# matchylabs/matchy

Hardware: AMD Instinct MI355X
Metric: log GB/s scanned (matchy match hot path, 100K IoCs) (higher is better)
Workload: dtype u8

## Files before the change

### matchy_amd/csrc/engine.cpp

```cpp
#include "engine.h"
#include "batch_reader.h"
#include "distinct.h"
#include "tally.h"
#include "unicode_lower.h"

#include <dlfcn.h>

#include <algorithm>
#include <chrono>
#include <cstdio>
#include <cstdlib>
#include <cstring>
#include <stdexcept>
#include <unordered_set>

#include "hashes.h"

namespace mxy {

void check_launch(const char* kernel) {
    const hipError_t e = hipGetLastError();
    if (e != hipSuccess) throw HipError{std::string("launch of ") + kernel + ": " + hipGetErrorString(e)};
}

// ... 191 lines not shown
                    launch_ip_leaf(ip_nodes.p, img.node_count, ip_l24.p, ctr.p + 1, (uint32_t)n_leaf, leaf_node.p, ip_leaf.p, nullptr);
                    MXY_HIP(hipDeviceSynchronize());
                    view.ip_leaf = ip_leaf.p;
                    bytes_uploaded += n_leaf * 256 * sizeof(uint2);
                }
                view.ip_l24 = ip_l24.p;
                bytes_uploaded += ((size_t)1 << 24) * sizeof(uint2);
                MXY_HIP(hipMemcpy(bm.data(), ip_bm24.p, bm.size() * 4, hipMemcpyDeviceToHost));
                have24 = true;
            } catch (const HipError&) {
                (void)hipGetLastError();
                ip_l24.free(); ip_leaf.free(); ip_bm24.free();
                view.ip_l24 = nullptr; view.ip_leaf = nullptr;
                std::fill(bm.begin(), bm.end(), 0u);
            }
        }
        if (!have24) {
            if (img.node_count > 0) {
                auto set_range = [&](uint32_t first, uint32_t count) {
                    for (uint32_t v = first; v < first + count;) {
                        if ((v & 31) == 0 && v + 32 <= first + count) { bm[v >> 5] = 0xFFFFFFFFu; v += 32; }
                        else { bm[v >> 5] |= 1u << (v & 31); ++v; }
                    }
                };
                struct Frame { uint32_t node, prefix, depth; };
                std::vector<Frame> st;
                st.push_back({v4_start, 0u, 0u});
                while (!st.empty()) {
                    const Frame f = st.back();
                    st.pop_back();
                    const uint2 nd = nodes[f.node];
                    for (uint32_t bit = 0; bit < 2; ++bit) {
                        const uint32_t rec = bit ? nd.y : nd.x;
                        const uint32_t depth = f.depth + 1;
                        const uint32_t prefix = f.prefix | (bit << (24 - depth));
                        if (rec == img.node_count) continue;
                        if (rec < img.node_count) {
                            if (depth == 24) set_range(prefix, 1);
                            else st.push_back({rec, prefix, depth});
                        } else if (rec - img.node_count >= 16) {
                            set_range(prefix, 1u << (24 - depth));
                        }
                    }
                }
            }
            ip_bm24.upload(bm);
        }
        view.ip_bm24 = ip_bm24.p;
        {
            uint64_t set = 0;
            for (uint32_t wv : bm) set += (uint64_t)__builtin_popcount(wv);
            view.ip_bm24_permille = (uint32_t)(set * 1000 / ((uint64_t)bm.size() * 32));
            view.ip_bm24_any = set ? 1u : 0u;
        }
        bytes_uploaded += bm.size() * 4;
    }
    if (img.has_literal) {
        std::vector<LitSlot> slots;
        uint32_t mask;
        img.build_lit_table(slots, mask);
        lit_slots.upload(slots);
        const uint8_t* pool = img.bytes.data() + img.lh_off + img.lh_strings_offset;
        std::vector<uint8_t> pv(pool, pool + img.lh_strings_size);
        lit_pool.upload(pv);
        {
            size_t bits = (size_t)1 << 22;
            size_t live = 0;
            for (const LitSlot& sl : slots) live += sl.str_off != 0xFFFFFFFFu;
            while (bits < live * 64 && bits < ((size_t)1 << 31)) bits <<= 1;
            std::vector<uint32_t> bm(bits / 32, 0u);
            const uint32_t bmask = (uint32_t)(bits - 1);
            for (const LitSlot& sl : slots) {
                if (sl.str_off == 0xFFFFFFFFu || (size_t)sl.str_off + 2 > pv.size()) continue;
                const size_t kl = (size_t)pv[sl.str_off] | ((size_t)pv[sl.str_off + 1] << 8);
                if ((size_t)sl.str_off + 2 + kl > pv.size()) continue;
                uint64_t lane[4] = {0, 0, 0, 0};
                memcpy(lane, pv.data() + sl.str_off + 2, std::min<size_t>(kl, 32));
                const uint32_t b = name_hash31(lane[0], lane[1], lane[2], lane[3], (uint32_t)kl) & bmask;
                bm[b >> 5] |= 1u << (b & 31);
            }
            lit_bm.upload(bm);
            view.lit_bm = lit_bm.p; view.lit_bm_mask = bmask;
            bytes_uploaded += bm.size() * 4;
        }
        uint32_t max_len = 0;
        for (const LitSlot& sl : slots)
            if (sl.str_off != 0xFFFFFFFFu && (size_t)sl.str_off + 2 <= pv.size()) max_len = std::max<uint32_t>(max_len, (uint32_t)pv[sl.str_off] | ((uint32_t)pv[sl.str_off + 1] << 8));
        view.lit_max_len = max_len;
        view.lit_slots = lit_slots.p; view.lit_mask = mask; view.has_literal = 1;
        view.lit_pool = lit_pool.p; view.lit_pool_size = img.lh_strings_size;
        bytes_uploaded += slots.size() * sizeof(LitSlot) + pv.size();
    }
    if (img.has_glob) {
        const uint8_t* pgp = img.bytes.data() + img.pg_off;
        std::vector<uint8_t> pv(pgp, pgp + img.pg_len);
        pv.resize((pv.size() + 3) & ~(size_t)3, 0);
        pg.upload(pv);
        std::vector<uint32_t> off, ids;
        img.build_lit2pat(off, ids);
        if (ids.empty()) ids.push_back(0);
        lit2pat_off.upload(off);
        lit2pat.upload(ids);
        auto r32 = [&](size_t o) { uint32_t v; memcpy(&v, pgp + o, 4); return v; };
        view.pg = pg.p; view.pg_len = (uint32_t)img.pg_len; view.has_glob = 1;
        view.ac_start = r32(20); view.ac_size = r32(24);
        view.patterns_off = r32(36); view.pattern_count = r32(32);
        uint32_t unaligned = r32(40) + r32(44);
        view.wild_off = unaligned + (8 - unaligned % 8) % 8;
        view.wild_count = r32(60);
        view.glob_seg_off = r32(104);
        view.glob_max_segs = 1;
        for (uint32_t pid = 0; pid < view.pattern_count; ++pid) view.glob_max_segs = std::max<uint32_t>(view.glob_max_segs, r32((size_t)view.glob_seg_off + (size_t)pid * 8 + 4) & 0xFFFFu);
        view.lit2pat_off = lit2pat_off.p; view.lit2pat = lit2pat.p; view.n_ac_lits = (uint32_t)off.size() - 1;
        {
            std::vector<uint32_t> nx, noff;
            std::vector<uint8_t> cls;
            uint32_t k = 0;
            size_t limit = (size_t)8 << 30;
            if (const char* env = getenv("MATCHY_AMD_DFA_MAX_MB")) limit = (size_t)atoll(env) << 20;
            bool alnum_literal = true;
            view.ac_alnum = 1;
            if (img.build_ac_dfa(nx, cls, k, noff, limit, &alnum_literal)) {
                view.ac_alnum = alnum_literal ? 1u : 0u;
                if (img.match_mode == 1) for (int c = 'A'; c <= 'Z'; ++c) cls[c] = cls[c + 32];
                dfa.upload(nx); dfa_node.upload(noff); dfa_cls.upload(cls);
                view.dfa = dfa.p; view.dfa_node = dfa_node.p; view.dfa_cls = dfa_cls.p; view.dfa_k = k;
                view.dfa_states = (uint32_t)noff.size();
                bytes_uploaded += nx.size() * 4 + noff.size() * 4 + 256;
            }
        }
        bytes_uploaded += pv.size() + (off.size() + ids.size()) * 4;
        if (view.dfa && view.wild_count == 0 && view.pattern_count && !getenv("MATCHY_AMD_NO_SUFFIX_FILTER")) {
            const bool ci_db = img.match_mode == 1;
            bool ok = true;
            int first = -1;
            uint32_t dots = 0;
            std::vector<std::pair<uint32_t, uint32_t>> lits;
            for (uint32_t pid = 0; pid < view.pattern_count && ok; ++pid) {
                const size_t io = (size_t)view.glob_seg_off + (size_t)pid * 8;
                const uint32_t firsth = r32(io), count = r32(io + 4) & 0xFFFFu;
                if (count != 2 || (size_t)firsth + 24 > img.pg_len) { ok = false; break; }
                const uint8_t* h0 = pgp + firsth;
                const uint8_t* h1 = pgp + firsth + 12;
                uint32_t dlen, doff;
                memcpy(&dlen, h1 + 4, 4); memcpy(&doff, h1 + 8, 4);
                if (h0[0] != 1 || h1[0] != 0 || (size_t)doff + dlen > img.pg_len) { ok = false; break; }
                if (dlen < 3) continue;
                const uint8_t* l = pgp + doff;
                const int fb = ci_db ? (int)ascii_lower1(l[0]) : (int)l[0];
                if (first < 0) first = fb;
                if (fb != first) { ok = false; break; }
                uint32_t d = 0;
                for (uint32_t k = 0; k < dlen; ++k) d += (ci_db ? ascii_lower1(l[k]) : l[k]) == (uint32_t)first;
                if (d > 32) { ok = false; break; }
                dots |= 1u << (d - 1);
                if (dlen <= 31) lits.push_back({doff, dlen});
            }
            if (ok && first >= 0 && __builtin_popcount(dots) <= 4) {
                size_t bits = (size_t)1 << 16;
                while (bits < lits.size() * 64 && bits < ((size_t)1 << 31)) bits <<= 1;
                std::vector<uint32_t> bm(bits / 32, 0u);
                const uint32_t bmask = (uint32_t)(bits - 1);
                for (auto& ol : lits) {
                    uint64_t lane[4] = {0, 0, 0, 0};
                    memcpy(lane, pgp + ol.first, ol.second);
                    if (ci_db) for (uint64_t& w : lane) w = ascii_lower8(w);
// ... 1053 lines not shown
```

### matchy_amd/csrc/engine.h

```cpp
#pragma once
#include <hip/hip_runtime.h>

#include <memory>
#include <mutex>
#include <string>
#include <vector>

#include "db_image.h"
#include "hip_owners.h"
#include "inflate.h"
#include "line_index.h"
#include "result_layout.h"
#include "scan_types.h"
#include "segments.h"

namespace mxy {

int anchor_blocks_per_cu();
int validate_blocks_per_cu(bool ac);
void launch_anchor(const TokParams& p, const DevDb& db, int grid, hipStream_t stream);
void launch_validate_dom(const TokParams& p, const DevDb& db, int grid, hipStream_t stream);
void launch_validate_misc(const TokParams& p, const DevDb& db, int grid, hipStream_t stream);
void launch_rare(const TokParams& p, const DevDb& db, int grid, hipStream_t stream);
void launch_lookup(const LookupParams& p, const DevDb& db, int grid, hipStream_t stream);
void launch_lookup_early_glob(const LookupParams& p, const DevDb& db, int grid, hipStream_t stream);
void launch_lookup_ip(const LookupParams& p, const DevDb& db, int grid, bool dense, hipStream_t stream);
void launch_lookup_spill(const LookupParams& p, const DevDb& db, hipStream_t stream);
uint32_t spill_threads();
void launch_ip_l24(const uint2* nodes, uint32_t node_count, uint32_t v4_start, uint2* l24, uint32_t* bm24, uint32_t* n_undecided, hipStream_t s);
void launch_ip_leaf(const uint2* nodes, uint32_t node_count, uint2* l24, uint32_t* next, uint32_t n_leaf, uint32_t* leaf_node, uint2* leaf, hipStream_t s);

class DistinctSet;
class HitTally;
struct TallyEntry;

struct PslHost {
    std::vector<std::string> suffixes;
    std::vector<PslSlot> slots;
    std::vector<uint8_t> pool;
    std::vector<uint32_t> bloom;
    std::vector<uint2> tld_tab;
    uint32_t mask = 0, max_tld_len = 0, max_suffix_len = 0;
    uint32_t tld_first[8] = {0};
    static const PslHost& get();
};

struct DeviceDb {
    int device = 0;
    DevDb view{};
    DevBuf<uint2> ip_nodes, ip_l1, ip_l24, ip_leaf;
    DevBuf<uint32_t> ip_bm24, lit_bm, sfx_bm;
    DevBuf<uint2> tld_tab;
    DevBuf<uint32_t> dfa, dfa_node;
    DevBuf<uint8_t> dfa_cls;
    DevBuf<LitSlot> lit_slots;
    DevBuf<uint8_t> lit_pool, pg, psl_pool;
    DevBuf<uint32_t> lit2pat_off, lit2pat, bloom;
    DevBuf<uint32_t> lit_offsets, glob_offsets;
    DevBuf<PslSlot> psl_slots;
    DevBuf<uint32_t> lc_map;
    DevBuf<uint2> lc_ign, lc_cased;
    uint32_t n_lit_offsets = 0, n_glob_offsets = 0;
    size_t bytes_uploaded = 0;
    void upload(const DbImage& img, int dev);
};

struct ScanTiming { float anchor_ms = 0, validate_ms = 0, rare_ms = 0, lookup_ms = 0, total_ms = 0; int slices = 1; };

enum HitMode { HITS_NONE = 0, HITS_FINAL = 1, HITS_RAW = 2 };

struct ScanOutput {
    std::vector<Candidate> cands;
    std::vector<Hit> hits;
    std::vector<uint32_t> ids;
    const FinalHit* fin = nullptr;
    const uint32_t* fin_ids = nullptr;
    const long long* fin_offs = nullptr;
    size_t n_fin = 0, n_fin_ids = 0;
    const uint2* c4 = nullptr;
    size_t n_c4 = 0;
    uint64_t lines = 0;
    uint32_t n_cand = 0, n_hits = 0;
    uint64_t by_type[IT_COUNT] = {0};
    bool has_lines = false;
    const LineRec* fin_lines = nullptr;
    const LineRec* c4_lines = nullptr;
    uint64_t lines_with_matches = 0;
    bool has_segments = false;
    const SegmentRec* segments = nullptr;
    size_t n_segments = 0;
    const uint32_t* seg_of_fin = nullptr;
    const uint32_t* seg_of_c4 = nullptr;
    std::vector<SegmentRec> seg_own;
    std::vector<uint32_t> seg_of_own;
};

namespace pins {
bool acquire(uintptr_t a, uintptr_t b);
void release(uintptr_t a, uintptr_t b);
int add_caller(const void* ptr, size_t bytes);
void remove_caller(const void* ptr);
}

template <class Hit, class Off, class OffOut>
void append_shifted(const Hit* hits, size_t n_hits, const uint32_t* ids, const Off* offs, size_t n_ids, uint32_t base,
                    std::vector<Hit>& all_hits, std::vector<uint32_t>& all_ids, std::vector<OffOut>& all_offs) {
    const uint32_t id_shift = (uint32_t)all_ids.size();
    for (size_t i = 0; i < n_hits; ++i) {
        Hit h = hits[i];
        h.start += base;
        if (h.kind == 3) h.value += id_shift;
        all_hits.push_back(h);
    }
    all_ids.insert(all_ids.end(), ids, ids + n_ids);
    all_offs.insert(all_offs.end(), offs, offs + n_ids);
}

struct ScanRequest {
    const uint8_t* ptr = nullptr;
    uint32_t len = 0;
    bool lookup = false;
    bool host_mirror = false;
    bool fork = false;
    int slices = 0;
    bool compact = false;
    bool lines = false;
};

template <class Line>
void append_shifted_lines(const Line* lines, size_t n, uint32_t base, uint32_t line_base, std::vector<Line>& all) {
    for (size_t i = 0; i < n; ++i) {
        Line l = lines[i];
        l.line += line_base; l.line_start += base; l.line_end += base;
        all.push_back(l);
// ... 155 lines not shown
```

### matchy_amd/csrc/hashes.h

```cpp
#pragma once
#include <cstddef>
#include <cstdint>

#if defined(__HIPCC__)
#include <hip/hip_runtime.h>
#define MXY_HD __host__ __device__ inline __attribute__((always_inline))
#else
#define MXY_HD inline
#endif

namespace mxy {

MXY_HD uint64_t rotl64(uint64_t x, int r) { return (x << r) | (x >> (64 - r)); }

template <class Fetch>
MXY_HD uint64_t xxh64_fetch(Fetch f, size_t len, uint64_t seed) {
    const uint64_t P1 = 11400714785074694791ULL, P2 = 14029467366897019727ULL, P3 = 1609587929392839161ULL,
                   P4 = 9650029242287828579ULL, P5 = 2870177450012600261ULL;
    auto rd64 = [&](size_t o) {
        uint64_t v = 0;
        for (int k = 7; k >= 0; --k) v = (v << 8) | (uint64_t)f(o + k);
        return v;
    };
    auto rd32 = [&](size_t o) {
// ... 50 lines not shown
            q += 32;
        } while (q <= limit);
        h = rotl64(v1, 1) + rotl64(v2, 7) + rotl64(v3, 12) + rotl64(v4, 18);
        h = merge(h, v1); h = merge(h, v2); h = merge(h, v3); h = merge(h, v4);
    } else {
        h = seed + P5;
    }
    h += (uint64_t)len;
    if (len >= 8) {
        const uint64_t last = rd64(len - 8);
        if (len < 32) {
            const uint64_t w0 = rd64(0), w1 = rd64(len >= 16 ? 8 : len - 8), w2 = rd64(len >= 24 ? 16 : len - 8);
            h ^= round(0, w0); h = rotl64(h, 27) * P1 + P4;
            if (len >= 16) { h ^= round(0, w1); h = rotl64(h, 27) * P1 + P4; }
            if (len >= 24) { h ^= round(0, w2); h = rotl64(h, 27) * P1 + P4; }
            q = len & ~(size_t)7;
        } else {
            while (q + 8 <= len) { h ^= round(0, rd64(q)); h = rotl64(h, 27) * P1 + P4; q += 8; }
        }
        size_t r = len - q;
        uint64_t tail = r ? last >> (8 * (8 - r)) : 0;
        if (r >= 4) { h ^= (tail & 0xFFFFFFFFull) * P1; h = rotl64(h, 23) * P2 + P3; tail >>= 32; r -= 4; }
        for (; r; --r) { h ^= (tail & 0xFF) * P5; h = rotl64(h, 11) * P1; tail >>= 8; }
    } else {
        if (q + 4 <= len) { h ^= rd32(q) * P1; h = rotl64(h, 23) * P2 + P3; q += 4; }
        while (q < len) { h ^= (uint64_t)(FOLD ? ascii_lower1(p[q]) : (uint32_t)p[q]) * P5; h = rotl64(h, 11) * P1; ++q; }
    }
    h ^= h >> 33; h *= P2; h ^= h >> 29; h *= P3; h ^= h >> 32;
    return h;
}

struct Xxh64Stream {
    static constexpr uint64_t P1 = 11400714785074694791ULL, P2 = 14029467366897019727ULL, P3 = 1609587929392839161ULL,
                              P4 = 9650029242287828579ULL, P5 = 2870177450012600261ULL;
    uint64_t v1, v2, v3, v4, lane[4] = {0, 0, 0, 0}, cur = 0, total = 0;
    uint32_t nlane = 0, ncur = 0;
    MXY_HD explicit Xxh64Stream(uint64_t seed) : v1(seed + P1 + P2), v2(seed + P2), v3(seed), v4(seed - P1) {}
    static MXY_HD uint64_t round(uint64_t acc, uint64_t in) { acc += in * P2; acc = rotl64(acc, 31); return acc * P1; }
    static MXY_HD uint64_t merge(uint64_t acc, uint64_t val) { val = round(0, val); acc ^= val; return acc * P1 + P4; }
    MXY_HD void push(uint32_t byte) {
        cur |= (uint64_t)(byte & 0xFF) << (8 * ncur);
        ++total;
        if (++ncur == 8) {
            lane[nlane] = cur; cur = 0; ncur = 0;
            if (++nlane == 4) {
                v1 = round(v1, lane[0]); v2 = round(v2, lane[1]); v3 = round(v3, lane[2]); v4 = round(v4, lane[3]);
                nlane = 0;
            }
        }
    }
    MXY_HD uint64_t finish(uint64_t seed) const {
        uint64_t h;
        if (total >= 32) {
            h = rotl64(v1, 1) + rotl64(v2, 7) + rotl64(v3, 12) + rotl64(v4, 18);
            h = merge(h, v1); h = merge(h, v2); h = merge(h, v3); h = merge(h, v4);
        } else {
            h = seed + P5;
        }
        h += total;
        for (uint32_t k = 0; k < nlane; ++k) { h ^= round(0, lane[k]); h = rotl64(h, 27) * P1 + P4; }
        uint64_t rest = cur;
        uint32_t n = ncur;
        if (n >= 4) { h ^= (rest & 0xFFFFFFFFull) * P1; h = rotl64(h, 23) * P2 + P3; rest >>= 32; n -= 4; }
        for (; n; --n) { h ^= (rest & 0xFF) * P5; h = rotl64(h, 11) * P1; rest >>= 8; }
        h ^= h >> 33; h *= P2; h ^= h >> 29; h *= P3; h ^= h >> 32;
        return h;
    }
};

MXY_HD uint32_t name_hash31(uint64_t l0, uint64_t l1, uint64_t l2, uint64_t l3, uint32_t n) {
    const uint64_t lane[4] = {l0, l1, l2, l3};
    uint32_t h = n * 0x9E3779B1u + 0x7F4A7C15u;
    for (int k = 0; k < 4; ++k) {
        const int rem = (int)n - 8 * k;
        const uint64_t m = rem >= 8 ? ~0ull : rem <= 0 ? 0ull : ((1ull << (8 * rem)) - 1ull);
        const uint64_t v = lane[k] & m;
        h = (h ^ (uint32_t)v) * 0x85EBCA6Bu; h ^= h >> 15;
        h = (h ^ (uint32_t)(v >> 32)) * 0xC2B2AE35u; h ^= h >> 13;
    }
    h *= 0x27D4EB2Fu; h ^= h >> 16;
    return h;
}

MXY_HD uint64_t fx_u32(uint32_t v) { return rotl64((uint64_t)v * 0xf1357aea2e62a9c5ULL, 26); }

constexpr uint32_t TLD_TAB_BITS = 11;
MXY_HD uint32_t tld_tab_slot(uint32_t lo, uint32_t hi24) { return ((lo ^ (hi24 * 0x9E3779B1u)) * 0x85EBCA6Bu) >> (32 - TLD_TAB_BITS); }

MXY_HD uint32_t tld_hash8(uint32_t lo, uint32_t hi) {
    uint32_t h = (lo * 0x9E3779B1u) ^ (hi * 0x85EBCA6Bu);
    h ^= h >> 16; h *= 0x7FEB352Du; h ^= h >> 15;
    return h;
}

MXY_HD uint64_t psl_hash_init() { return 0xcbf29ce484222325ULL; }
MXY_HD uint64_t psl_hash_step(uint64_t h, uint8_t b) { return (h ^ b) * 0x100000001b3ULL; }
MXY_HD uint64_t psl_hash_finish(uint64_t h) { h ^= h >> 29; h *= 0xbf58476d1ce4e5b9ULL; h ^= h >> 32; return h; }

}
```

### matchy_amd/csrc/scan_types.h

```cpp
#pragma once
#include <hip/hip_runtime.h>

#include <cstdint>

namespace mxy {

enum ItemType : uint8_t {
    IT_DOMAIN = 0, IT_EMAIL = 1, IT_IPV4 = 2, IT_IPV6 = 3, IT_MD5 = 4, IT_SHA1 = 5, IT_SHA256 = 6,
    IT_SHA384 = 7, IT_SHA512 = 8, IT_BITCOIN = 9, IT_ETHEREUM = 10, IT_MONERO = 11, IT_COUNT = 12
};
enum ExtractFlags : uint32_t {
    EX_DOMAINS = 1, EX_EMAILS = 2, EX_IPV4 = 4, EX_IPV6 = 8, EX_HASHES = 16, EX_BITCOIN = 32, EX_ETHEREUM = 64,
    EX_MONERO = 128, EX_ALL = 255
};

struct Candidate {
    uint32_t start;
    uint32_t len_type;
    uint32_t v4;
    uint32_t pad;
};
constexpr uint32_t CAND_NO_GLOB = 1, CAND_GLOB = 2;

enum RareKind : uint32_t { RARE_V6 = 0, RARE_AT = 1, RARE_TOK = 2, HEAVY_B58 = 3, HEAVY_BECH32 = 4, HEAVY_ETH = 5, HEAVY_XMR = 6, RARE_DOM = 7 };
struct RareAnchor {
    uint32_t pos;
    uint32_t len_kind;
};

struct Hit {
    uint32_t cand;
    uint32_t a;
    uint32_t ids_off;
    uint16_t n_globs;
    uint8_t kind;
    uint8_t prefix_len;
    uint32_t start;
    uint32_t len_type;
};

struct LitSlot { uint64_t hash; uint32_t str_off; uint32_t pattern_id; };
struct PslSlot { uint64_t hash; uint32_t off; uint32_t len; };

struct DevDb {
    const uint2* ip_nodes;
    uint32_t ip_bm24_permille;
    uint32_t ip_bm24_any;
    const uint32_t* ip_bm24;
    const uint2* ip_l1;
    const uint2* ip_l24;
    const uint2* ip_leaf;
    uint32_t node_count;
    uint32_t ip_version;
    uint32_t v4_start_node;
    uint32_t has_ip;
    const LitSlot* lit_slots;
    uint32_t lit_mask;
    uint32_t has_literal;
    const uint32_t* lit_bm;
    uint32_t lit_bm_mask;
    const uint8_t* lit_pool;
    uint32_t lit_pool_size;
    uint32_t lit_max_len;
    const uint8_t* pg;
    uint32_t pg_len;
    uint32_t has_glob;
    uint32_t ac_start, ac_size;
    uint32_t patterns_off, pattern_count;
    uint32_t wild_off, wild_count;
    uint32_t glob_seg_off;
    uint32_t glob_max_segs;
    const uint32_t* dfa;
    const uint8_t* dfa_cls;
    const uint32_t* dfa_node;
    uint32_t dfa_k;
    uint32_t dfa_states;
    const uint32_t* sfx_bm;
    uint32_t sfx_mask;
    uint32_t sfx_first;
    uint32_t sfx_dots;
    const uint32_t* lit2pat_off;
    const uint32_t* lit2pat;
    uint32_t n_ac_lits;
    uint32_t ac_alnum;
    const PslSlot* psl_slots;
    uint32_t psl_mask;
    const uint8_t* psl_pool;
    const uint32_t* tld_bloom;
    uint32_t max_tld_len;
    uint32_t max_suffix_len;
    const uint2* tld_tab;
    uint32_t tld_first[8];
    uint32_t ci;
    const uint32_t* lc_map;
    uint32_t lc_n;
    const uint2* lc_ign;
    uint32_t lc_n_ign;
    const uint2* lc_cased;
    uint32_t lc_n_cased;
};

constexpr uint32_t DFA_LDS_ENTRIES = 8192;
constexpr uint32_t DFA_LDS_ENTRIES_GLOB = 2048;
constexpr uint32_t DFA_LDS_ENTRIES_VAL = 2048;
constexpr uint32_t TLD_BLOOM_BITS = 32768;
constexpr uint32_t TLD_BLOOM_WORDS = TLD_BLOOM_BITS / 32;

struct ScanCounters {
    alignas(128) unsigned long long lines;
    uint32_t cand_true;
    uint32_t hits_true;
    uint32_t error;
    uint32_t reserved0;
    alignas(128) uint32_t n_cand;
    alignas(128) uint32_t n_cand_a;
    alignas(128) uint32_t n_cand_m;
    uint32_t n_cand_d;
    uint32_t n_cand_r;
    alignas(128) uint32_t n_dom;
    alignas(128) uint32_t n_rare;
    alignas(128) uint32_t n_rare_dom;
    alignas(128) uint32_t n_tok;
    alignas(128) uint32_t n_heavy;
    alignas(128) uint32_t n_hits;
    uint32_t n_ids;
    alignas(128) uint32_t n_final;
    uint32_t n_final_ids;
    uint32_t n_c4;
    alignas(128) uint32_t chains_done;
    uint32_t arrive_wgs[3];
    alignas(128) uint32_t n_glob_work;
    uint32_t n_glob_work_d;
    uint32_t n_spill;
};

struct FinalHit {
    uint32_t start;
    uint32_t len_type;
    uint32_t value;
    uint8_t kind, prefix_len;
    uint16_t n_ids;
};

// ... 119 lines not shown
```

### matchy_amd/csrc/validate_kernels.hip

```cpp
#include <hip/hip_runtime.h>

#include <cstdlib>

#include "hashes.h"
#include "scan_types.h"

#include "device_shared.h"
#include "domain_planes.h"

namespace mxy {


struct BackReader {
    const uint8_t* p;
    uint32_t pos;
    uint32_t cb;
    uint32_t k;
    uint64_t cur, nxt;
    __device__ __forceinline__ static uint64_t load8(const uint8_t* a) { uint64_t v; __builtin_memcpy(&v, a, 8); return v; }
    __device__ __forceinline__ void init(const uint8_t* base, uint32_t q) {
        p = base; pos = q; cb = 0; k = 0; cur = 0; nxt = 0;
        if (q >= 16) { cb = q - 8; k = 8; cur = load8(p + cb); nxt = load8(p + cb - 8); }
    }
    __device__ __forceinline__ uint32_t next() {
// ... 662 lines not shown
    for (int i = 0; i < NL; ++i) {
#pragma unroll
        for (int bb = 0; bb < 4; ++bb) {
            const uint32_t j = 4 * i + bb;
            if (j < nbytes) dec[zeros + nbytes - 1 - j] = (uint8_t)(L[i] >> (8 * bb));
        }
    }
    return zeros + nbytes;
}
__device__ bool val_btc_base58(const uint8_t* s, uint32_t n, uint8_t* dec) {
    const uint32_t dl = d_base58_decode<12>(s, n, dec);
    if (dl < 5) return false;
    Sha256 h1, h2;
    h1.hash(dec, dl - 4);
    uint32_t w[16];
#pragma unroll
    for (int i = 0; i < 8; ++i) w[i] = h1.h[i];
    w[8] = 0x80000000u;
#pragma unroll
    for (int i = 9; i < 15; ++i) w[i] = 0;
    w[15] = 256;
    h2.init();
    h2.block(w);
    const uint32_t chk = ((uint32_t)dec[dl - 4] << 24) | ((uint32_t)dec[dl - 3] << 16) | ((uint32_t)dec[dl - 2] << 8) | dec[dl - 1];
    return h2.h[0] == chk;
}
__device__ bool val_monero(const uint8_t* s, uint32_t n, uint8_t* dec) {
    const uint32_t dl = d_base58_decode<21>(s, n, dec);
    if (dl < 5) return false;
    uint64_t h[4];
    d_keccak256_1blk(dec, dl - 4, h);
    const uint32_t chk = (uint32_t)dec[dl - 4] | ((uint32_t)dec[dl - 3] << 8) | ((uint32_t)dec[dl - 2] << 16) | ((uint32_t)dec[dl - 1] << 24);
    return (uint32_t)h[0] == chk;
}
__device__ int d_bech32_val(uint32_t c) {
    const char* CS = "qpzry9x8gf2tvdw0s3jn54khce6mua7l";
    for (int i = 0; i < 32; ++i) if ((uint32_t)CS[i] == c) return i;
    return -1;
}
__device__ bool val_btc_bech32(const uint8_t* s, uint32_t n) {
    if (n < 3 + 6) return false;
    auto step = [](uint32_t chk, uint32_t v) {
        const uint32_t GEN[5] = {0x3b6a57b2, 0x26508e6d, 0x1ea119fa, 0x3d4233dd, 0x2a1462b3};
        uint32_t top = chk >> 25;
        chk = ((chk & 0x1ffffff) << 5) ^ v;
        for (int i = 0; i < 5; ++i) if ((top >> i) & 1) chk ^= GEN[i];
        return chk;
    };
    uint32_t chk = 1;
    chk = step(chk, 'b' >> 5); chk = step(chk, 'c' >> 5); chk = step(chk, 0); chk = step(chk, 'b' & 31); chk = step(chk, 'c' & 31);
    for (uint32_t k = 3; k < n; ++k) {
        int v = d_bech32_val(s[k]);
        if (v < 0) return false;
        chk = step(chk, (uint32_t)v);
    }
    return chk == 1 || chk == 0x2bc830a3u;
}
__device__ bool val_eth(const uint8_t* a, uint8_t* lower) {
    bool all_lower = true, all_upper = true;
    for (int i = 0; i < 40; ++i) {
        uint32_t c = a[2 + i];
        if (!d_is_hex(c)) return false;
        if (d_is_alpha(c)) { if (c >= 'a') all_upper = false; else all_lower = false; }
        lower[i] = (uint8_t)d_lower(c);
    }
    if (all_lower || all_upper) return true;
    uint64_t h[4];
    d_keccak256_1blk(lower, 40, h);
    for (int i = 0; i < 40; ++i) {
        uint32_t c = a[2 + i];
        if (d_is_alpha(c)) {
            const uint32_t byte = (uint32_t)(h[i >> 4] >> (8 * ((i >> 1) & 7))) & 0xFF;
            const uint32_t nib = (i & 1) ? (byte & 0x0f) : (byte >> 4);
            if ((c < 'a') != (nib >= 8)) return false;
        }
    }
    return true;
}

template <int MODE>
__global__ __launch_bounds__(256) void k_validate_dom(TokParams p, DevDb db) {
    constexpr bool AC = MODE == 1, SFX = MODE == 2;
    __shared__ uint2 tldtab[1u << TLD_TAB_BITS];
    __shared__ __attribute__((aligned(16))) uint32_t strbuf[256][8];
    __shared__ uint8_t dcls[AC ? 256 : 4];
    __shared__ uint32_t drows[AC ? DFA_LDS_ENTRIES_VAL : 1];
    for (uint32_t i = threadIdx.x; i < (1u << TLD_TAB_BITS); i += blockDim.x) tldtab[i] = db.tld_tab[i];
    DfaView dv{dcls, drows, 0};
    if constexpr (AC) dv = dfa_stage<DFA_LDS_ENTRIES_VAL>(db, dcls, drows);
    __syncthreads();
    ChunkWriter<Candidate, CAND_CHUNK> cw_dense;
    __shared__ Candidate wb_cand[4][64];
    BufferedWriter<Candidate> cw(wb_cand[threadIdx.x >> 6]);
    __shared__ RareAnchor wb_slow[4][64];
    BufferedWriter<RareAnchor> sw(wb_slow[threadIdx.x >> 6]);
    const Candidate SC{0, 0xFFFFFFFFu, 0, 0};
    const uint32_t stride = gridDim.x * blockDim.x;
    const uint32_t nd = min(p.counters->n_dom, p.dom_cap);
    struct Rec { uint32_t j; uint32_t c[8]; };
    auto load_rec = [&](uint32_t i, Rec& r) {
        const uint32_t ic = i < nd ? i : 0u;
        const uint32_t j = p.dom_list[dom_plane_index(ic, 0)];
#pragma unroll
        for (int k = 0; k < 8; ++k) r.c[k] = p.dom_list[dom_plane_index(ic, 1 + k)];
        r.j = i < nd ? j : 0xFFFFFFFFu;
    };
    Rec cur, nxt;
    load_rec(blockIdx.x * blockDim.x + threadIdx.x, cur);
    {
        uint32_t g = cur.j;
#pragma unroll
        for (int k = 0; k < 8; ++k) g ^= cur.c[k];
        asm volatile("" ::"v"(g));
    }
    uint32_t pend_start = 0, pend_lt = 0, pend_word = 0xFFFFFFFFu, pend_bit = 0, n_valid = 0;
    uint32_t pend_sw[SFX ? 4 : 1] = {0}, pend_sb[SFX ? 4 : 1] = {0};
    bool pend = false, pend_over = false;
    uint32_t* sb = strbuf[threadIdx.x];
    auto queue_glob = [&](uint32_t b, uint32_t n) {
        if (!p.glob_work_d) return;
        const uint32_t lane = lane_id();
        const bool g = lane < n && b + lane < p.cand_cap && cw.buf[lane].pad == CAND_GLOB;
        const uint64_t m = __ballot(g);
        if (!m) return;
        uint32_t wb = 0;
        if (lane == 0) wb = atomicAdd(&p.counters->n_glob_work_d, (uint32_t)__popcll(m));
        wb = __builtin_amdgcn_readfirstlane(wb);
        const uint32_t slot = wb + mbcnt64(m);
        if (g && slot < p.glob_work_d_cap) p.glob_work_d[slot] = b + lane;
    };
    auto emit_pending = [&]() {
        if (!p.filter_lit) { cw_dense.append(pend, Candidate{pend_start, pend_lt, 0u, 0u}, p.cands, p.cand_cap, p.n_cand, SC); return; }
        bool lit = (pend_word >> pend_bit) & 1;
        uint32_t flag = 0;
        if constexpr (SFX) {
            bool g = pend_over;
#pragma unroll
            for (int q = 0; q < 4; ++q) g = g || ((pend_sw[q] >> pend_sb[q]) & 1);
            flag = g ? CAND_GLOB : CAND_NO_GLOB;
            lit = lit || g;
        }
        if constexpr (AC) flag = pend_over ? CAND_GLOB : CAND_NO_GLOB;
        if constexpr (AC || SFX) cw.append_then(pend && lit, Candidate{pend_start, pend_lt, 0u, flag}, p.cands, p.cand_cap, p.n_cand, queue_glob);
        else cw.append(pend && lit, Candidate{pend_start, pend_lt, 0u, flag}, p.cands, p.cand_cap, p.n_cand);
    };
    for (uint32_t base = blockIdx.x * blockDim.x; base < nd; base += stride) {
        const uint32_t i = base + threadIdx.x;
        emit_pending();
        pend = false;
        load_rec(i + stride, nxt);
        bool slow = false;
        if (cur.j != 0xFFFFFFFFu) {
            uint32_t s = 0, e = 0;
            int r = 2;
            if (!(cur.j & 0x80000000u)) r = domain_rules(tldtab, p.min_labels, cur.j, cur.c, s, e);
            slow = r == 2;
            if (r == 1) {
                pend_start = s; pend_lt = (e - s) | ((uint32_t)IT_DOMAIN << 24); pend = true;
                pend_word = 0xFFFFFFFFu; pend_bit = 0;
                n_valid += 1;
                if (p.filter_lit) {
                    *reinterpret_cast<uint4*>(sb) = make_uint4(cur.c[0], cur.c[1], cur.c[2], cur.c[3]);
                    *reinterpret_cast<uint4*>(sb + 4) = make_uint4(cur.c[4], cur.c[5], cur.c[6], cur.c[7]);
                    const uint32_t o = 24 - (cur.j - s), n = e - s;
                    const uint32_t i0 = o >> 2, sh = o & 3;
                    uint32_t wd[9];
#pragma unroll
                    for (int k = 0; k < 9; ++k) wd[k] = (i0 + k) < 8 ? sb[(i0 + k) & 7] : 0u;
                    uint64_t ln[4];
#pragma unroll
                    for (int k = 0; k < 4; ++k)
                        ln[k] = (uint64_t)__builtin_amdgcn_alignbyte(wd[2 * k + 1], wd[2 * k], sh) |
                                ((uint64_t)__builtin_amdgcn_alignbyte(wd[2 * k + 2], wd[2 * k + 1], sh) << 32);
                    if (db.ci) {
#pragma unroll
                        for (int k = 0; k < 4; ++k) ln[k] = ascii_lower8(ln[k]);
                    }
                    const uint32_t b = name_hash31(ln[0], ln[1], ln[2], ln[3], n) & db.lit_bm_mask;
                    pend_word = db.lit_bm ? db.lit_bm[b >> 5] : 0u;
                    pend_bit = b & 31;
                    if constexpr (SFX) {
                        const uint64_t fb = 0x0101010101010101ull * db.sfx_first;
                        uint32_t M = 0;
#pragma unroll
                        for (int k = 0; k < 4; ++k) {
                            const uint64_t x = ln[k] ^ fb;
                            const uint64_t z = ~(((x & 0x7F7F7F7F7F7F7F7Full) + 0x7F7F7F7F7F7F7F7Full) | x) & 0x8080808080808080ull;
                            const uint32_t lo = (uint32_t)z >> 7, hi = (uint32_t)(z >> 32) >> 7;
                            M |= ((((lo * 0x01020408u) >> 24) & 0xFu) | ((((hi * 0x01020408u) >> 24) & 0xFu) << 4)) << (8 * k);
                        }
                        M &= n >= 32 ? 0xFFFFFFFFu : ((1u << n) - 1u);
                        pend_over = false;
                        uint32_t dm = db.sfx_dots;
#pragma unroll
                        for (int q = 0; q < 4; ++q) {
                            pend_sw[q] = 0; pend_sb[q] = 0;
                            if (dm) {
                                const uint32_t d = (uint32_t)__builtin_ctz(dm) + 1;
                                dm &= dm - 1;
                                uint32_t m = M;
                                for (uint32_t j = 1; j < d; ++j) m &= ~(m ? (0x80000000u >> __builtin_clz(m)) : 0u);
                                if (m) {
                                    const uint32_t kk = 31u - (uint32_t)__builtin_clz(m), sl = n - kk;
                                    if (sl >= 3) {
                                        const uint32_t o2 = o + kk, j0 = o2 >> 2, s2 = o2 & 3;
                                        uint32_t w2[9];
#pragma unroll
                                        for (int k = 0; k < 9; ++k) w2[k] = (j0 + k) < 8 ? sb[(j0 + k) & 7] : 0u;
                                        uint64_t l2[4];
#pragma unroll
                                        for (int k = 0; k < 4; ++k)
                                            l2[k] = (uint64_t)__builtin_amdgcn_alignbyte(w2[2 * k + 1], w2[2 * k], s2) |
                                                    ((uint64_t)__builtin_amdgcn_alignbyte(w2[2 * k + 2], w2[2 * k + 1], s2) << 32);
                                        if (db.ci) {
#pragma unroll
                                            for (int k = 0; k < 4; ++k) l2[k] = ascii_lower8(l2[k]);
                                        }
                                        const uint32_t b2 = name_hash31(l2[0], l2[1], l2[2], l2[3], sl) & db.sfx_mask;
                                        pend_sw[q] = db.sfx_bm[b2 >> 5];
                                        pend_sb[q] = b2 & 31;
                                    }
                                }
                            }
                        }
                    }
                    if constexpr (AC) {
                        uint32_t st = 0, any = 0;
#pragma unroll
                        for (int k = 0; k < 31; ++k) {
                            const uint32_t c = dcls[(uint32_t)(ln[k >> 3] >> (8 * (k & 7))) & 0xFF];
                            if ((uint32_t)k < n) {
                                const uint32_t t = st < dv.lds_states ? drows[st * db.dfa_k + c] : db.dfa[(size_t)st * db.dfa_k + c];
                                st = t & 0x7FFFFFFFu;
                                any |= t;
                            }
                        }
                        pend_over = (any >> 31) != 0;
                        if (pend_over) { pend_word = 0xFFFFFFFFu; pend_bit = 0; }
                    }
                }
            }
        }
        sw.append(slow, RareAnchor{cur.j & 0x7FFFFFFFu, (uint32_t)RARE_DOM}, p.rare_dom, p.rare_dom_cap, &p.counters->n_rare_dom);
        cur = nxt;
    }
    emit_pending();
    if constexpr (AC || SFX) cw.flush_then(p.cands, p.cand_cap, p.n_cand, queue_glob);
    else cw.flush(p.cands, p.cand_cap, p.n_cand);
    cw_dense.pad_rest(p.cands, p.cand_cap, SC);
    sw.flush(p.rare_dom, p.rare_dom_cap, &p.counters->n_rare_dom);
#pragma unroll
    for (int off = 32; off > 0; off >>= 1) n_valid += __shfl_down(n_valid, off);
    if (lane_id() == 0 && n_valid) atomicAdd(&p.counters->cand_true, n_valid);
}

__device__ __forceinline__ bool lit_bm_may_hit(const DevDb& db, const LogView& lg, uint32_t s, uint32_t n, bool ascii) {
    uint64_t l[4] = {0, 0, 0, 0};
    if (s + 32 <= lg.len) {
#pragma unroll
        for (int k = 0; k < 4; ++k) __builtin_memcpy(&l[k], lg.p + s + 8 * k, 8);
    } else {
        for (uint32_t k = 0; k < 32 && s + k < lg.len; ++k) l[k >> 3] |= (uint64_t)lg.p[s + k] << (8 * (k & 7));
    }
    if (db.ci) {
        if (!ascii) {
            if (n > 32) return true;
            uint64_t high = 0;
#pragma unroll
            for (int k = 0; k < 4; ++k) {
                const int rem = (int)n - 8 * k;
                const uint64_t m = rem >= 8 ? ~0ull : (rem <= 0 ? 0ull : ((1ull << (8 * rem)) - 1ull));
                high |= l[k] & m & 0x8080808080808080ull;
            }
            if (high) return true;
        }
#pragma unroll
        for (int k = 0; k < 4; ++k) l[k] = ascii_lower8(l[k]);
    }
    const uint32_t b = name_hash31(l[0], l[1], l[2], l[3], n) & db.lit_bm_mask;
    return ((db.lit_bm[b >> 5] >> (b & 31)) & 1u) != 0;
}

template <uint32_t VM>
__global__ __launch_bounds__(256) void k_validate(TokParams p, DevDb db) {
    constexpr bool MISC = (VM & 1u) != 0, DOM = (VM & 2u) != 0, TOK = (VM & 4u) != 0;
    __shared__ uint32_t bloom[DOM ? TLD_BLOOM_WORDS : 1];
    constexpr bool TLD_LDS = DOM && (MISC || TOK);
    __shared__ uint2 tldtab[TLD_LDS ? (1u << TLD_TAB_BITS) : 1];
    const uint2* const tldtab_p = TLD_LDS ? tldtab : db.tld_tab;
    constexpr uint32_t WIN = MISC ? 80 : 64;
    constexpr uint32_t WIN_BACK = WIN - (MISC ? 32 : 16);
    __shared__ __attribute__((aligned(16))) uint8_t winbuf[(MISC || DOM) ? 256 * WIN : 16];
    if constexpr (DOM && !MISC && !TOK) {
        if (blockIdx.x * blockDim.x >= min(p.counters->n_rare_dom, p.rare_dom_cap)) return;
    }
    if constexpr (TOK && !MISC && !DOM) {
        if (blockIdx.x * blockDim.x >= min(p.counters->n_tok, p.tok_cap)) return;
    }
    if constexpr (DOM) {
        for (uint32_t i = threadIdx.x; i < TLD_BLOOM_WORDS; i += blockDim.x) bloom[i] = db.tld_bloom[i];
        if constexpr (TLD_LDS) for (uint32_t i = threadIdx.x; i < (1u << TLD_TAB_BITS); i += blockDim.x) tldtab[i] = db.tld_tab[i];
        __syncthreads();
    }
    LogView lg{p.log, p.len};
    __shared__ Candidate wb_cand[4][64];
    BufferedWriter<Candidate> cw(wb_cand[threadIdx.x >> 6]);
    const uint32_t stride = gridDim.x * blockDim.x;
    __shared__ RareAnchor wb_heavy[4][64];
    BufferedWriter<RareAnchor> hw(wb_heavy[threadIdx.x >> 6]);
    const uint32_t nt = TOK ? min(p.counters->n_tok, p.tok_cap) : 0u;
    uint32_t unlisted_tok = 0;
    const bool lit_only = p.filter_lit && !db.has_glob && db.lit_bm != nullptr;
    const bool tok_filter = p.filter_lit && db.lit_bm != nullptr && (!db.has_glob || !db.ac_alnum);
    RareAnchor ra_next{0, 0xFF};
    if (TOK && blockIdx.x * blockDim.x + threadIdx.x < nt) ra_next = p.tok[blockIdx.x * blockDim.x + threadIdx.x];
    for (uint32_t base = blockIdx.x * blockDim.x; base < nt; base += stride) {
        const RareAnchor ra = ra_next;
        ra_next = RareAnchor{0, 0xFF};
        if (base + stride + threadIdx.x < nt) ra_next = p.tok[base + stride + threadIdx.x];
        const bool live = (ra.len_kind & 0xFF) == RARE_TOK;
        const uint32_t tl = ra.len_kind >> 8;
// ... 323 lines not shown
```

Before: 2336.

## Prefilter domain candidates with a fragment-keyed bitmap instead of full-name hash

Builds a second bloom-style bitmap keyed on a short fragment of each literal: up to 8 bytes before the last dot, the final label, and the total length. The dom validate kernel hashes this fragment from registers it already holds instead of staging the token through LDS and realigning the full name. In the plain mode the per-thread LDS string buffer shrinks to one row, which may raise occupancy. The trade-off is a weaker filter with more false positives passed downstream, and the bit index is packed into pend_lt, which assumes those bits are otherwise unused.

```diff
diff --git a/matchy_amd/csrc/engine.cpp b/matchy_amd/csrc/engine.cpp
--- a/matchy_amd/csrc/engine.cpp
+++ b/matchy_amd/csrc/engine.cpp
@@ -297,6 +297,27 @@
             lit_bm.upload(bm);
             view.lit_bm = lit_bm.p; view.lit_bm_mask = bmask;
             bytes_uploaded += bm.size() * 4;
+            std::vector<NameFragment> frags;
+            for (const LitSlot& sl : slots) {
+                if (sl.str_off == 0xFFFFFFFFu || (size_t)sl.str_off + 2 > pv.size()) continue;
+                const size_t kl = (size_t)pv[sl.str_off] | ((size_t)pv[sl.str_off + 1] << 8);
+                if ((size_t)sl.str_off + 2 + kl > pv.size()) continue;
+                NameFragment f;
+                if (name_fragment_key(pv.data() + sl.str_off + 2, kl, f)) frags.push_back(f);
+            }
+            if (!frags.empty()) {
+                size_t dbits = (size_t)1 << 22;
+                while (dbits < frags.size() * 64 && dbits < ((size_t)1 << 31)) dbits <<= 1;
+                std::vector<uint32_t> dbm(dbits / 32, 0u);
+                const uint32_t dmask = (uint32_t)(dbits - 1);
+                for (const NameFragment& f : frags) {
+                    const uint32_t b = name_frag_hash(f) & dmask;
+                    dbm[b >> 5] |= 1u << (b & 31);
+                }
+                dom_bm.upload(dbm);
+                view.dom_bm = dom_bm.p; view.dom_bm_mask = dmask;
+                bytes_uploaded += dbm.size() * 4;
+            }
         }
         uint32_t max_len = 0;
         for (const LitSlot& sl : slots)
diff --git a/matchy_amd/csrc/engine.h b/matchy_amd/csrc/engine.h
--- a/matchy_amd/csrc/engine.h
+++ b/matchy_amd/csrc/engine.h
@@ -49,7 +49,7 @@
     int device = 0;
     DevDb view{};
     DevBuf<uint2> ip_nodes, ip_l1, ip_l24, ip_leaf;
-    DevBuf<uint32_t> ip_bm24, lit_bm, sfx_bm;
+    DevBuf<uint32_t> ip_bm24, lit_bm, dom_bm, sfx_bm;
     DevBuf<uint2> tld_tab;
     DevBuf<uint32_t> dfa, dfa_node;
     DevBuf<uint8_t> dfa_cls;
diff --git a/matchy_amd/csrc/hashes.h b/matchy_amd/csrc/hashes.h
--- a/matchy_amd/csrc/hashes.h
+++ b/matchy_amd/csrc/hashes.h
@@ -156,6 +156,47 @@
     return h;
 }
 
+struct NameFragment {
+    uint64_t pre;
+    uint64_t lab;
+    uint32_t n;
+};
+
+MXY_HD NameFragment name_fragment_ctx(uint64_t pre8, uint64_t lab8, uint32_t consumed, uint32_t ll, bool fold) {
+    const uint32_t k = consumed < 8u ? consumed : 8u;
+    NameFragment f;
+    f.pre = pre8 >> (8u * (8u - k));
+    f.lab = lab8 & ((1ull << (8u * ll)) - 1ull);
+    if (fold) { f.pre = ascii_lower8(f.pre); f.lab = ascii_lower8(f.lab); }
+    f.n = consumed + ll;
+    return f;
+}
+
+MXY_HD bool name_fragment_key(const uint8_t* key, size_t len, NameFragment& f) {
+    if (len > 31 || len < 2) return false;
+    size_t d = len;
+    while (d > 0 && key[d - 1] != '.') --d;
+    if (d == 0) return false;
+    const size_t ll = len - d;
+    if (ll < 1 || ll > 7) return false;
+    const size_t k = d < 8 ? d : 8;
+    f.pre = 0; f.lab = 0;
+    for (size_t q = 0; q < k; ++q) f.pre |= (uint64_t)key[d - k + q] << (8 * q);
+    for (size_t q = 0; q < ll; ++q) f.lab |= (uint64_t)key[d + q] << (8 * q);
+    f.n = (uint32_t)len;
+    return true;
+}
+
+MXY_HD uint32_t name_frag_hash(const NameFragment& f) {
+    uint32_t h = f.n * 0x9E3779B1u + 0x7F4A7C15u;
+    h = (h ^ (uint32_t)f.pre) * 0x85EBCA6Bu; h ^= h >> 15;
+    h = (h ^ (uint32_t)(f.pre >> 32)) * 0xC2B2AE35u; h ^= h >> 13;
+    h = (h ^ (uint32_t)f.lab) * 0x85EBCA6Bu; h ^= h >> 15;
+    h = (h ^ (uint32_t)(f.lab >> 32)) * 0xC2B2AE35u; h ^= h >> 13;
+    h *= 0x27D4EB2Fu; h ^= h >> 16;
+    return h;
+}
+
 MXY_HD uint64_t fx_u32(uint32_t v) { return rotl64((uint64_t)v * 0xf1357aea2e62a9c5ULL, 26); }
 
 constexpr uint32_t TLD_TAB_BITS = 11;
diff --git a/matchy_amd/csrc/scan_types.h b/matchy_amd/csrc/scan_types.h
--- a/matchy_amd/csrc/scan_types.h
+++ b/matchy_amd/csrc/scan_types.h
@@ -58,7 +58,9 @@
     uint32_t lit_mask;
     uint32_t has_literal;
     const uint32_t* lit_bm;
+    const uint32_t* dom_bm;
     uint32_t lit_bm_mask;
+    uint32_t dom_bm_mask;
     const uint8_t* lit_pool;
     uint32_t lit_pool_size;
     uint32_t lit_max_len;
diff --git a/matchy_amd/csrc/validate_kernels.hip b/matchy_amd/csrc/validate_kernels.hip
--- a/matchy_amd/csrc/validate_kernels.hip
+++ b/matchy_amd/csrc/validate_kernels.hip
@@ -768,7 +768,7 @@
 __global__ __launch_bounds__(256) void k_validate_dom(TokParams p, DevDb db) {
     constexpr bool AC = MODE == 1, SFX = MODE == 2;
     __shared__ uint2 tldtab[1u << TLD_TAB_BITS];
-    __shared__ __attribute__((aligned(16))) uint32_t strbuf[256][8];
+    __shared__ __attribute__((aligned(16))) uint32_t strbuf[(AC || SFX) ? 256 : 1][8];
     __shared__ uint8_t dcls[AC ? 256 : 4];
     __shared__ uint32_t drows[AC ? DFA_LDS_ENTRIES_VAL : 1];
     for (uint32_t i = threadIdx.x; i < (1u << TLD_TAB_BITS); i += blockDim.x) tldtab[i] = db.tld_tab[i];
@@ -802,7 +802,7 @@
     uint32_t pend_start = 0, pend_lt = 0, pend_word = 0xFFFFFFFFu, pend_bit = 0, n_valid = 0;
     uint32_t pend_sw[SFX ? 4 : 1] = {0}, pend_sb[SFX ? 4 : 1] = {0};
     bool pend = false, pend_over = false;
-    uint32_t* sb = strbuf[threadIdx.x];
+    [[maybe_unused]] uint32_t* sb = strbuf[(AC || SFX) ? threadIdx.x : 0];
     auto queue_glob = [&](uint32_t b, uint32_t n) {
         if (!p.glob_work_d) return;
         const uint32_t lane = lane_id();
@@ -818,6 +818,7 @@
     auto emit_pending = [&]() {
         if (!p.filter_lit) { cw_dense.append(pend, Candidate{pend_start, pend_lt, 0u, 0u}, p.cands, p.cand_cap, p.n_cand, SC); return; }
         bool lit = (pend_word >> pend_bit) & 1;
+        if constexpr (AC || SFX) { lit = (pend_word >> ((pend_lt >> 8) & 31)) & 1; pend_lt &= 0xFF0000FFu; }
         uint32_t flag = 0;
         if constexpr (SFX) {
             bool g = pend_over;
@@ -826,7 +827,7 @@
             flag = g ? CAND_GLOB : CAND_NO_GLOB;
             lit = lit || g;
         }
-        if constexpr (AC) flag = pend_over ? CAND_GLOB : CAND_NO_GLOB;
+        if constexpr (AC) { flag = pend_over ? CAND_GLOB : CAND_NO_GLOB; lit = lit || pend_over; }
         if constexpr (AC || SFX) cw.append_then(pend && lit, Candidate{pend_start, pend_lt, 0u, flag}, p.cands, p.cand_cap, p.n_cand, queue_glob);
         else cw.append(pend && lit, Candidate{pend_start, pend_lt, 0u, flag}, p.cands, p.cand_cap, p.n_cand);
     };
@@ -846,25 +847,32 @@
                 pend_word = 0xFFFFFFFFu; pend_bit = 0;
                 n_valid += 1;
                 if (p.filter_lit) {
-                    *reinterpret_cast<uint4*>(sb) = make_uint4(cur.c[0], cur.c[1], cur.c[2], cur.c[3]);
-                    *reinterpret_cast<uint4*>(sb + 4) = make_uint4(cur.c[4], cur.c[5], cur.c[6], cur.c[7]);
-                    const uint32_t o = 24 - (cur.j - s), n = e - s;
-                    const uint32_t i0 = o >> 2, sh = o & 3;
-                    uint32_t wd[9];
-#pragma unroll
-                    for (int k = 0; k < 9; ++k) wd[k] = (i0 + k) < 8 ? sb[(i0 + k) & 7] : 0u;
-                    uint64_t ln[4];
-#pragma unroll
-                    for (int k = 0; k < 4; ++k)
-                        ln[k] = (uint64_t)__builtin_amdgcn_alignbyte(wd[2 * k + 1], wd[2 * k], sh) |
-                                ((uint64_t)__builtin_amdgcn_alignbyte(wd[2 * k + 2], wd[2 * k + 1], sh) << 32);
-                    if (db.ci) {
-#pragma unroll
-                        for (int k = 0; k < 4; ++k) ln[k] = ascii_lower8(ln[k]);
+                    const uint32_t consumed = cur.j - s, n = e - s;
+                    if constexpr (!AC) {
+                        const NameFragment fr = name_fragment_ctx(((uint64_t)cur.c[5] << 32) | cur.c[4], ((uint64_t)cur.c[7] << 32) | cur.c[6],
+                                                                  consumed, e - cur.j, db.ci != 0);
+                        const uint32_t b = name_frag_hash(fr) & db.dom_bm_mask;
+                        pend_word = db.dom_bm ? db.dom_bm[b >> 5] : 0u;
+                        if constexpr (AC || SFX) pend_lt |= (b & 31) << 8; else pend_bit = b & 31;
                     }
-                    const uint32_t b = name_hash31(ln[0], ln[1], ln[2], ln[3], n) & db.lit_bm_mask;
-                    pend_word = db.lit_bm ? db.lit_bm[b >> 5] : 0u;
-                    pend_bit = b & 31;
+                    [[maybe_unused]] const uint32_t o = 24 - consumed;
+                    [[maybe_unused]] uint64_t ln[4];
+                    if constexpr (AC || SFX) {
+                        *reinterpret_cast<uint4*>(sb) = make_uint4(cur.c[0], cur.c[1], cur.c[2], cur.c[3]);
+                        *reinterpret_cast<uint4*>(sb + 4) = make_uint4(cur.c[4], cur.c[5], cur.c[6], cur.c[7]);
+                        const uint32_t i0 = o >> 2, sh = o & 3;
+                        uint32_t wd[9];
+#pragma unroll
+                        for (int k = 0; k < 9; ++k) wd[k] = (i0 + k) < 8 ? sb[(i0 + k) & 7] : 0u;
+#pragma unroll
+                        for (int k = 0; k < 4; ++k)
+                            ln[k] = (uint64_t)__builtin_amdgcn_alignbyte(wd[2 * k + 1], wd[2 * k], sh) |
+                                    ((uint64_t)__builtin_amdgcn_alignbyte(wd[2 * k + 2], wd[2 * k + 1], sh) << 32);
+                        if (db.ci) {
+#pragma unroll
+                            for (int k = 0; k < 4; ++k) ln[k] = ascii_lower8(ln[k]);
+                        }
+                    }
                     if constexpr (SFX) {
                         const uint64_t fb = 0x0101010101010101ull * db.sfx_first;
                         uint32_t M = 0;
@@ -922,7 +930,13 @@
                             }
                         }
                         pend_over = (any >> 31) != 0;
-                        if (pend_over) { pend_word = 0xFFFFFFFFu; pend_bit = 0; }
+                    }
+                    if constexpr (AC) {
+                        const NameFragment fr = name_fragment_ctx(((uint64_t)cur.c[5] << 32) | cur.c[4], ((uint64_t)cur.c[7] << 32) | cur.c[6],
+                                                                  consumed, e - cur.j, db.ci != 0);
+                        const uint32_t b = name_frag_hash(fr) & db.dom_bm_mask;
+                        pend_word = db.dom_bm ? db.dom_bm[b >> 5] : 0u;
+                        if constexpr (AC || SFX) pend_lt |= (b & 31) << 8; else pend_bit = b & 31;
                     }
                 }
             }
```

Result: no change. 2342 (median of 5 runs) (+0.2%).
